# YuejiangDong/PPEA-Depth

Hardware: AMD Instinct MI355X
Metric: training img/s at 640x192 RepLKNet-31B (higher is better)
Workload: dtype bf16; 1 GPU; RepLKNet-31B Stage-1 640x192, 12 frame triplets/GPU, process_batch + backward + grad all-reduce + Adam; global_batch=12, per_gpu_batch=12, parallelism=dp1, use_checkpoint=BN-stat replay, no recompute (288 GB HBM), launch=whole step captured in one hipGraph

## Files before the change

### include/ppea_depth.h

```cpp
#ifndef PPEA_DEPTH_H
#define PPEA_DEPTH_H

#include <stdint.h>

#ifdef __cplusplus
extern "C" {
#endif

#define PPEA_ERR_UNSUPPORTED (-1)
#define PPEA_ERR_ARG (-2)

int ppea_abi_version(void);

int ppea_timestamp(void* slot, void* stream);

int ppea_dwconv_lk_fwd_f32(const float* x, const float* w_big, const float* w_small,
                           float* y_big, float* y_small,
                           int N, int C, int H, int W, int K, int KS, void* stream);
int ppea_dwconv_lk_fwd_bf16(const uint16_t* x, const float* w_big, const float* w_small,
                            uint16_t* y_big, uint16_t* y_small,
                            int N, int C, int H, int W, int K, int KS, void* stream);

int ppea_dwconv_lk_bwd_data_f32(const float* dy_big, const float* dy_small,
                                const float* w_big, const float* w_small, float* dx,
// ... 207 lines not shown
int ppea_ssim_l1_bwd_f32(const float* pred, const float* target, const float* d_out,
                         long dout_bstride, float* d_pred, int B, int C, int H, int W,
                         float alpha, void* stream);

int ppea_smooth_num_partials(void);
int ppea_smooth_fwd_f32(const float* disp, const float* img, float* partials,
                        int B, int C, int H, int W, void* stream);
int ppea_smooth_bwd_f32(const float* disp, const float* img, float gx, float gy, float* d_disp,
                        int B, int C, int H, int W, void* stream);

int ppea_loss_select_f32(const float* reproj, const float* identity, const float* warped_m1,
                         const float* warped_p1, const float* noise, float* sel,
                         uint8_t* src_idx, int64_t* frame_idx, int64_t* auto_idx,
                         int B, int C, int H, int W, int selec_reproj, void* stream);

int ppea_loss_tail_blocks(long total);
int ppea_loss_tail_fwd_f32(const float* sel, const int64_t* auto_idx, const float* cons, const float* aug, const float* multi,
                           const float* mono, float* mask, float* target, float* partial, float* out, int B, int H, int W,
                           int is_multi, void* stream);
int ppea_loss_tail_bwd_f32(const float* mask, const uint8_t* src, const float* out, const float* g_rl, const float* g_con,
                           const float* multi, const float* mono, float* d_reproj, float* d_multi, int B, int H, int W,
                           void* stream);

long ppea_conv_packed_bytes(int Cout, int Cin, int R, int S, int flip);
int ppea_conv_pack_weights(const void* w, int w_is_bf16, void* packed, int Cout, int Cin, int R, int S, int flip,
                           void* stream);
int ppea_conv_nhwc_bf16(const void* x, const void* w_packed, const void* bias, int bias_bf16, void* y,
                        int N, int H, int W, int Cin, int Cout, int R, int S, int stride, int pad, int reflect, int dil,
                        int Ho, int Wo, int act, int out_nchw, void* stream);
long ppea_conv_wgrad_workspace_bytes(int N, int Cin, int Cout, int R, int S, int stride, int Ho, int Wo);
int ppea_conv_wgrad_nhwc_bf16(const void* dz, const void* x, void* dw, int dw_bf16, void* workspace,
                              int N, int H, int W, int Cin, int Cout, int R, int S, int stride, int pad, int reflect,
                              int Ho, int Wo, void* stream);
int ppea_image_to_nhwc_bf16(const float* x, void* y, int N, int C, int H, int W, int Cp, float sub, float div,
                            void* stream);

int ppea_conv2d_f32_fwd(const float* x, const long* xs, const float* w, const float* bias, float* y, const long* ys, int N,
                        int Cin, int H, int W, int Cout, int R, int S, int stride, int pad, void* stream);
int ppea_conv2d_f32_dgrad(const float* dy, const long* dys, const float* w, float* dx, const long* dxs, int N, int Cin, int H,
                          int W, int Cout, int R, int S, int stride, int pad, int Ho, int Wo, void* stream);
long ppea_conv2d_f32_wgrad_workspace_bytes(int N, int Cin, int Cout, int R, int S, int Ho, int Wo);
int ppea_conv2d_f32_wgrad(const float* x, const long* xs, const float* dy, const long* dys, float* dw, float* workspace, int N,
                          int Cin, int H, int W, int Cout, int R, int S, int stride, int pad, int Ho, int Wo, void* stream);
int ppea_conv2d_bf16_fwd(const void* x, const long* xs, const void* w, const float* bias, void* y, const long* ys, int N,
                         int Cin, int H, int W, int Cout, int R, int S, int stride, int pad, void* stream);
int ppea_conv2d_bf16_dgrad(const void* dy, const long* dys, const void* w, void* dx, const long* dxs, int N, int Cin, int H,
                           int W, int Cout, int R, int S, int stride, int pad, int Ho, int Wo, void* stream);
int ppea_conv2d_bf16_wgrad(const void* x, const long* xs, const void* dy, const long* dys, float* dw, float* workspace, int N,
                           int Cin, int H, int W, int Cout, int R, int S, int stride, int pad, int Ho, int Wo, void* stream);

int ppea_nhwc_maxpool3x3s2_fwd_f32(const void* x, void* y, void* idx, int N, int H, int W, int C, void* stream);
int ppea_nhwc_maxpool3x3s2_fwd_bf16(const void* x, void* y, void* idx, int N, int H, int W, int C, void* stream);
int ppea_nhwc_maxpool3x3s2_bwd_f32(const void* dy, const void* idx, void* dx, int N, int H, int W, int C, void* stream);
int ppea_nhwc_maxpool3x3s2_bwd_bf16(const void* dy, const void* idx, void* dx, int N, int H, int W, int C, void* stream);

long ppea_conv_image_packed_bytes(int Cout, int K);
int ppea_conv_image_pack_weights(const void* w, int w_is_bf16, void* packed, int Cout, int Cin, int K, void* stream);
int ppea_conv_image_bf16(const void* x, const void* w_packed, void* y, int N, int H, int W, int Cout, int K, int stride,
                         int pad, int Ho, int Wo, int out_nchw, void* stream);
long ppea_conv_image_wgrad_workspace_bytes(int N, int Cout, int K, int Ho, int Wo);
int ppea_conv_image_wgrad_bf16(const void* dz, const void* x, void* dw, int dw_bf16, void* workspace, int N, int H, int W,
                               int Cin, int Cout, int K, int stride, int pad, int Ho, int Wo, void* stream);

int ppea_cost_volume_multi_fwd_f32(const float* cur, const float* lookup, const float* P, const float* inv_K,
                                   const float* bins, const int32_t* skip, float* cost, int B, int F, int C, int h, int w,
                                   int D, float eps, void* stream);
// ... 76 lines not shown
```

### ppea-depth_amd/csrc/common.h

```cpp
#pragma once
#include <hip/hip_runtime.h>
#include <stdint.h>

#define PPEA_ABI_VERSION 19
#define PPEA_ERR_UNSUPPORTED (-1)
#define PPEA_ERR_ARG (-2)
#define WAVE 64

__device__ __forceinline__ float bf16_to_f32(uint16_t v) {
    return __uint_as_float(((uint32_t)v) << 16);
}
__device__ __forceinline__ uint16_t f32_to_bf16(float f) {
    uint32_t u = __float_as_uint(f);
    if ((u & 0x7fffffffu) > 0x7f800000u) return (uint16_t)((u >> 16) | 0x40u);
    u += 0x7fffu + ((u >> 16) & 1u);
    return (uint16_t)(u >> 16);
}

template <typename T> __device__ __forceinline__ float ld_f32(const T* p);
template <> __device__ __forceinline__ float ld_f32<float>(const float* p) { return *p; }
template <> __device__ __forceinline__ float ld_f32<uint16_t>(const uint16_t* p) { return bf16_to_f32(*p); }
template <typename T> __device__ __forceinline__ void st_f32(T* p, float v);
template <> __device__ __forceinline__ void st_f32<float>(float* p, float v) { *p = v; }
template <> __device__ __forceinline__ void st_f32<uint16_t>(uint16_t* p, float v) { *p = f32_to_bf16(v); }

__device__ __forceinline__ float wave_sum(float v) {
#pragma unroll
    for (int o = 32; o > 0; o >>= 1) v += __shfl_xor(v, o, WAVE);
    return v;
}

static inline int launch_status() { return (int)hipGetLastError(); }
```

### ppea-depth_amd/csrc/conv_nhwc.hip

```cpp
#include "common.h"
#include <cstdlib>

namespace {

typedef __attribute__((ext_vector_type(8))) __bf16 bf16x8;
typedef __attribute__((ext_vector_type(4))) float f32x4;

constexpr int TILE_PX = 128;
constexpr int PITCH = 64;
__device__ __forceinline__ int swz_chunk(int row) { return ((row >> 2) & 1) << 1; }
constexpr int halo_cap(int stride, int ks) {
    return ks <= 3 ? (stride == 1 ? 4 * 66 : 9 * 65) : (stride == 1 ? 14 * 22 : 21 * 37);
}

__device__ __forceinline__ float bf2f(uint16_t v) { return __builtin_bit_cast(float, (uint32_t)v << 16); }
__device__ __forceinline__ uint16_t f2bf(float v) { return __builtin_bit_cast(uint16_t, (__bf16)v); }

struct ConvArgs {
    const uint16_t* x;
    const uint16_t* w;
    const void* bias;
    uint16_t* y;
    int N, H, W, Cin, CinP, Cout, stride, pad, reflect, dil, Ho, Wo, act, bias_bf16;
    int TR, TC, tiles_x, tiles_y;
};

enum { ACT_NONE = 0, ACT_RELU = 1, ACT_ELU = 2, ACT_SIGMOID = 3 };

template <int BN, int WM, int WN, int STRIDE, bool OUT_NCHW, int KS, int RPS = 1>
__global__ __launch_bounds__(256, 2) void conv_nhwc_kernel(const ConvArgs a) {
    static_assert(WM * WN == 4, "four waves");
    static_assert(RPS == 1 || RPS == KS, "one filter row or all of them per step");
    constexpr int MAX_A = (halo_cap(STRIDE, KS) * 4 + 255) / 256, MAX_B = (RPS * KS * BN * 4 + 255) / 256;
    constexpr int MT = 8 / WM;
    constexpr int NT = BN / 16 / WN;
    extern __shared__ __attribute__((aligned(16))) uint8_t lds[];

    const int TR = a.TR, TC = a.TC;
    const int HALO_H = (TR - 1) * STRIDE + KS, HALO_W = (TC - 1) * STRIDE + KS;
    const int halo_px = HALO_H * HALO_W;
    uint8_t* ldsA = lds;
    uint8_t* ldsB = lds + ((halo_px * PITCH + 127) / 128) * 128;

    const int tid = threadIdx.x, lane = tid & 63, wave = tid >> 6;
    const int wm = wave / WN, wn = wave % WN;
    const int g = lane >> 4, li = lane & 15;
    const int co0 = blockIdx.x * BN;
    int t = blockIdx.y;
    const int tx = t % a.tiles_x; t /= a.tiles_x;
    const int ty = t % a.tiles_y;
    const int n = t / a.tiles_y;
    const int oh0 = ty * TR, ow0 = tx * TC;
    const int ih0 = oh0 * STRIDE - a.pad, iw0 = ow0 * STRIDE - a.pad;
    const int Hl = (a.H - 1) * a.dil + 1, Wl = (a.W - 1) * a.dil + 1;
    const uint16_t* xn = a.x + (long)n * a.H * a.W * a.Cin;

    f32x4 acc[MT][NT];
#pragma unroll
    for (int i = 0; i < MT; ++i)
#pragma unroll
        for (int j = 0; j < NT; ++j) acc[i][j] = {0.f, 0.f, 0.f, 0.f};

    const int a_chunks = halo_px * 4;
    int a_src[MAX_A];
// ... 32 lines not shown
#pragma unroll
        for (int c = 0; c < MAX_A; ++c) {
            const int q = tid + c * 256;
            if (q < a_chunks) *reinterpret_cast<uint4*>(ldsA + (q >> 2) * PITCH + (((q & 3) ^ swz_chunk(q >> 2)) << 4)) = a_reg[c];
        }
    };
    auto load_b = [&](int c0, int r) {
#pragma unroll
        for (int c = 0; c < MAX_B; ++c) {
            const int q = tid + c * 256;
            if (q < b_chunks) {
                const int row = q >> 2;
                const int s = row / BN, co = co0 + row % BN;
                b_reg[c] = co < a.Cout ? *reinterpret_cast<const uint4*>(
                                             a.w + ((long)(r * KS + s) * a.Cout + co) * a.CinP + c0 + (q & 3) * 8)
                                       : make_uint4(0, 0, 0, 0);
            }
        }
    };
    auto store_b = [&]() {
#pragma unroll
        for (int c = 0; c < MAX_B; ++c) {
            const int q = tid + c * 256;
            if (q < b_chunks) *reinterpret_cast<uint4*>(ldsB + (q >> 2) * PITCH + (((q & 3) ^ swz_chunk(q >> 2)) << 4)) = b_reg[c];
        }
    };

    int a_px[MT];
#pragma unroll
    for (int i = 0; i < MT; ++i) {
        int m = (wm * MT + i) * 16 + li;
        if (m >= TR * TC) m = 0;
        a_px[i] = (m / TC) * STRIDE * HALO_W + (m % TC) * STRIDE;
    }
    const int b_off = (wn * NT * 16 + li) * PITCH + ((g ^ swz_chunk(li)) << 4);

    constexpr int SPS = KS / RPS;
    const int steps = (a.CinP / 32) * SPS;
    load_a(0);
    load_b(0, 0);
    for (int st = 0; st < steps; ++st) {
        const int r0 = (st % SPS) * RPS;
        __syncthreads();
        store_b();
        if (r0 == 0) store_a();
        __syncthreads();
        const int nxt = st + 1;
        if (nxt < steps) {
            load_b((nxt / SPS) * 32, (nxt % SPS) * RPS);
            if ((nxt % SPS) == 0) load_a((nxt / SPS) * 32);
        }
#pragma unroll
        for (int rr = 0; rr < RPS; ++rr) {
            const int r = r0 + rr;
#pragma unroll
            for (int s = 0; s < KS; ++s) {
                bf16x8 af[MT], bfr[NT];
#pragma unroll
                for (int i = 0; i < MT; ++i) {
                    const int px = a_px[i] + r * HALO_W + s;
                    af[i] = __builtin_bit_cast(bf16x8, *reinterpret_cast<const uint4*>(ldsA + px * PITCH + ((g ^ swz_chunk(px)) << 4)));
                }
#pragma unroll
                for (int j = 0; j < NT; ++j)
                    bfr[j] = __builtin_bit_cast(bf16x8, *reinterpret_cast<const uint4*>(ldsB + b_off + ((rr * KS + s) * BN + j * 16) * PITCH));
#pragma unroll
                for (int i = 0; i < MT; ++i)
#pragma unroll
                    for (int j = 0; j < NT; ++j) {
                        if constexpr (OUT_NCHW)
                            acc[i][j] = __builtin_amdgcn_mfma_f32_16x16x32_bf16(af[i], bfr[j], acc[i][j], 0, 0, 0);
                        else
                            acc[i][j] = __builtin_amdgcn_mfma_f32_16x16x32_bf16(bfr[j], af[i], acc[i][j], 0, 0, 0);
                    }
            }
        }
    }

    auto activate = [&](float v) -> float {
        switch (a.act) {
            case ACT_RELU: return v > 0.f ? v : 0.f;
            case ACT_ELU: return v > 0.f ? v : (__expf(v) - 1.f);
            case ACT_SIGMOID: return 1.f / (1.f + __expf(-v));
            default: return v;
        }
    };
    auto bias_at = [&](int co) -> float {
        if (a.bias == nullptr) return 0.f;
        return a.bias_bf16 ? bf2f(reinterpret_cast<const uint16_t*>(a.bias)[co]) : reinterpret_cast<const float*>(a.bias)[co];
    };
#pragma unroll
    for (int i = 0; i < MT; ++i) {
#pragma unroll
        for (int j = 0; j < NT; ++j) {
            const int cb = co0 + (wn * NT + j) * 16;
            if constexpr (OUT_NCHW) {
                const int m0 = (wm * MT + i) * 16 + 4 * g;
                const int oh = oh0 + m0 / TC, ow = ow0 + m0 % TC, co = cb + li;
                if (m0 >= TR * TC || oh >= a.Ho || co >= a.Cout || ow >= a.Wo) continue;
                const float bv = bias_at(co);
                uint16_t* dst = a.y + (((long)n * a.Cout + co) * a.Ho + oh) * a.Wo + ow;
                uint16_t v[4];
#pragma unroll
                for (int e = 0; e < 4; ++e) v[e] = f2bf(activate(acc[i][j][e] + bv));
                if (ow + 3 < a.Wo && (a.Wo & 3) == 0) {
                    *reinterpret_cast<uint2*>(dst) = make_uint2(v[0] | ((uint32_t)v[1] << 16), v[2] | ((uint32_t)v[3] << 16));
                } else {
// ... 8 lines not shown
                uint16_t* dst = a.y + (((long)n * a.Ho + oh) * a.Wo + ow) * a.Cout + co;
                uint16_t v[4];
#pragma unroll
                for (int e = 0; e < 4; ++e) v[e] = (co + e < a.Cout) ? f2bf(activate(acc[i][j][e] + bias_at(co + e))) : 0;
                if (co + 3 < a.Cout && (a.Cout & 3) == 0) {
                    *reinterpret_cast<uint2*>(dst) = make_uint2(v[0] | ((uint32_t)v[1] << 16), v[2] | ((uint32_t)v[3] << 16));
                } else {
#pragma unroll
                    for (int e = 0; e < 4; ++e)
                        if (co + e < a.Cout) dst[e] = v[e];
                }
            }
        }
    }
}

void pick_tile(ConvArgs& a, int stride, int ks, bool nchw) {
    int best_tr = 8, best_tc = 16;
    long best = (long)((a.Ho + 7) / 8) * ((a.Wo + 15) / 16);
    const int cand[4][2] = {{4, 32}, {2, 64}, {a.Wo <= 64 ? TILE_PX / a.Wo : 0, a.Wo}, {0, 0}};
    for (int c = 0; c < 3; ++c) {
        int tr = cand[c][0], tc = cand[c][1];
        if (tr <= 0 || tc <= 0) continue;
        if (tr > a.Ho) tr = a.Ho;
        if (nchw && (tc & 3)) continue;
        if (((tr - 1) * stride + ks) * ((tc - 1) * stride + ks) > halo_cap(stride, ks)) continue;
        const long tiles = (long)((a.Ho + tr - 1) / tr) * ((a.Wo + tc - 1) / tc);
        if (tiles < best) { best = tiles; best_tr = tr; best_tc = tc; }
    }
    a.TR = best_tr; a.TC = best_tc;
    a.tiles_x = (a.Wo + a.TC - 1) / a.TC; a.tiles_y = (a.Ho + a.TR - 1) / a.TR;
}

template <int BN, int WM, int WN, int STRIDE, bool NCHW, int KS, int RPS = 1>
int launch_conv(const ConvArgs& a, hipStream_t st) {
    const int halo_px = ((a.TR - 1) * STRIDE + KS) * ((a.TC - 1) * STRIDE + KS);
    if (halo_px > halo_cap(STRIDE, KS)) return PPEA_ERR_UNSUPPORTED;
    if constexpr (RPS == 1 && KS == 3 && BN <= 64) {
        static const bool one_row = getenv("PPEA_CONV_RPS") != nullptr && getenv("PPEA_CONV_RPS")[0] == '1';
        if (!one_row && a.CinP >= 256) return launch_conv<BN, WM, WN, STRIDE, NCHW, KS, KS>(a, st);
    }
    const size_t smem = (size_t)((halo_px * PITCH + 127) / 128) * 128 + (size_t)RPS * KS * BN * PITCH;
    if (smem > 160 * 1024) return PPEA_ERR_UNSUPPORTED;
    auto kern = conv_nhwc_kernel<BN, WM, WN, STRIDE, NCHW, KS, RPS>;
    if (smem > 64 * 1024) {
        hipError_t e = hipFuncSetAttribute(reinterpret_cast<const void*>(kern), hipFuncAttributeMaxDynamicSharedMemorySize, (int)smem);
        if (e != hipSuccess) return (int)e;
    }
    const dim3 grid((a.Cout + BN - 1) / BN, (unsigned)((long)a.tiles_x * a.tiles_y * a.N));
    hipLaunchKernelGGL(kern, grid, dim3(256), smem, st, a);
    return launch_status();
}

template <int STRIDE, bool NCHW, int KS>
int dispatch_bn(const ConvArgs& a, hipStream_t st) {
    const long tiles = (long)a.tiles_x * a.tiles_y * a.N;
    if constexpr (KS <= 3) {
        if (a.Cout > 64 && tiles * ((a.Cout + 127) / 128) >= 512 && !(KS == 3 && a.CinP >= 256))
            return launch_conv<128, 2, 2, STRIDE, NCHW, KS>(a, st);
    }
    static const bool no_narrow = getenv("PPEA_CONV_NO_NARROW") != nullptr;
    if (a.Cout > 32 && (no_narrow || tiles * ((a.Cout + 63) / 64) >= 256)) return launch_conv<64, 2, 2, STRIDE, NCHW, KS>(a, st);
    return launch_conv<32, 4, 1, STRIDE, NCHW, KS>(a, st);
}

template <int STRIDE, bool NCHW>
int dispatch_conv(ConvArgs& a, int ks, hipStream_t st) {
    pick_tile(a, STRIDE, ks, NCHW);
    switch (ks) {
        case 1: return dispatch_bn<STRIDE, NCHW, 1>(a, st);
        case 3: return dispatch_bn<STRIDE, NCHW, 3>(a, st);
        case 7: return dispatch_bn<STRIDE, NCHW, 7>(a, st);
    }
    return PPEA_ERR_UNSUPPORTED;
}

template <int NTC, int SL>
__global__ __launch_bounds__(256) void conv3x3_resident_kernel(const ConvArgs a) {
    constexpr int TR = 8, TC = 16, HALO_W = TC + 2, HALO_PX = (TR + 2) * HALO_W;
    constexpr int CO_ROWS = NTC * 16, MT = 2;
    constexpr int W_BYTES = SL * 9 * CO_ROWS * PITCH, H_BYTES = SL * HALO_PX * PITCH;
    constexpr int A_CHUNKS = SL * HALO_PX * 4, MAX_A = (A_CHUNKS + 255) / 256;
    extern __shared__ __attribute__((aligned(16))) uint8_t lds[];
    uint8_t* ldsW = lds;
    uint8_t* ldsH = lds + W_BYTES;

    const int tid = threadIdx.x, lane = tid & 63, wave = tid >> 6;
    const int g = lane >> 4, li = lane & 15;
    const int tiles = a.tiles_x * a.tiles_y * a.N;

    for (int q = tid; q < SL * 9 * CO_ROWS * 4; q += 256) {
        const int c = q & 3, row = q >> 2;
        const int co = row % CO_ROWS, st = row / CO_ROWS, tap = st % 9, sl = st / 9;
        uint4 v = make_uint4(0, 0, 0, 0);
        if (co < a.Cout) v = *reinterpret_cast<const uint4*>(a.w + ((long)tap * a.Cout + co) * a.CinP + sl * 32 + c * 8);
        *reinterpret_cast<uint4*>(ldsW + row * PITCH + ((c ^ swz_chunk(co)) << 4)) = v;
    }

    typedef __attribute__((ext_vector_type(4))) int i32x4;
    const unsigned long xb = (unsigned long)a.x;
    const unsigned nbytes = (unsigned)((long)a.N * a.H * a.W * a.Cin * 2);
    i32x4 rs;
    rs[0] = __builtin_amdgcn_readfirstlane((int)(unsigned)(xb & 0xffffffffu));
    rs[1] = __builtin_amdgcn_readfirstlane((int)(unsigned)(xb >> 32));
    rs[2] = __builtin_amdgcn_readfirstlane((int)nbytes);
    rs[3] = __builtin_amdgcn_readfirstlane(0x00020000);
    typedef __attribute__((ext_vector_type(4))) unsigned int u32x4;
    u32x4 a_reg[MAX_A];
    auto load_halo = [&](int t) {
        const int tx = t % a.tiles_x, ty = (t / a.tiles_x) % a.tiles_y, n = t / (a.tiles_x * a.tiles_y);
// ... 29 lines not shown
            if (q < A_CHUNKS) {
                const int c = q & 3, rest = q >> 2, px = rest % HALO_PX;
                *reinterpret_cast<u32x4*>(buf + rest * PITCH + ((c ^ swz_chunk(px)) << 4)) = a_reg[k];
            }
        }
    };

    int a_px[MT];
#pragma unroll
    for (int i = 0; i < MT; ++i) a_px[i] = (wave * MT + i) * HALO_W + li;
    const int b_off = li * PITCH + ((g ^ swz_chunk(li)) << 4);

    float bias_r[NTC][4];
#pragma unroll
    for (int j = 0; j < NTC; ++j)
#pragma unroll
        for (int e = 0; e < 4; ++e) {
            const int co = j * 16 + 4 * g + e;
            bias_r[j][e] = 0.f;
            if (a.bias != nullptr && co < a.Cout)
                bias_r[j][e] = a.bias_bf16 ? bf2f(reinterpret_cast<const uint16_t*>(a.bias)[co])
                                           : reinterpret_cast<const float*>(a.bias)[co];
        }

    int t = blockIdx.x;
    load_halo(t);
    halo_wait();
    store_halo(ldsH);
    __syncthreads();
    int cur = 0;
    for (; t < tiles; t += gridDim.x) {
        const int tn = t + gridDim.x;
        if (tn < tiles) load_halo(tn);
        const uint8_t* hb = ldsH + cur * H_BYTES;
        f32x4 acc[MT][NTC];
#pragma unroll
        for (int i = 0; i < MT; ++i)
#pragma unroll
            for (int j = 0; j < NTC; ++j) acc[i][j] = {0.f, 0.f, 0.f, 0.f};
#pragma unroll
        for (int sl = 0; sl < SL; ++sl)
#pragma unroll
            for (int r = 0; r < 3; ++r)
#pragma unroll
                for (int s3 = 0; s3 < 3; ++s3) {
                    bf16x8 af[MT], bfr[NTC];
#pragma unroll
                    for (int i = 0; i < MT; ++i) {
                        const int px = a_px[i] + r * HALO_W + s3;
                        af[i] = __builtin_bit_cast(bf16x8, *reinterpret_cast<const uint4*>(
                                                               hb + (sl * HALO_PX + px) * PITCH + ((g ^ swz_chunk(px)) << 4)));
                    }
#pragma unroll
                    for (int j = 0; j < NTC; ++j)
                        bfr[j] = __builtin_bit_cast(bf16x8, *reinterpret_cast<const uint4*>(
                                                                ldsW + b_off + (((sl * 9 + r * 3 + s3) * NTC + j) * 16) * PITCH));
#pragma unroll
                    for (int i = 0; i < MT; ++i)
#pragma unroll
                        for (int j = 0; j < NTC; ++j)
                            acc[i][j] = __builtin_amdgcn_mfma_f32_16x16x32_bf16(bfr[j], af[i], acc[i][j], 0, 0, 0);
                }
        const int tx = t % a.tiles_x, ty = (t / a.tiles_x) % a.tiles_y, n = t / (a.tiles_x * a.tiles_y);
#pragma unroll
        for (int i = 0; i < MT; ++i) {
            const int oh = ty * TR + wave * MT + i, ow = tx * TC + li;
            if (oh >= a.Ho || ow >= a.Wo) continue;
            uint16_t* row = a.y + (((long)n * a.Ho + oh) * a.Wo + ow) * a.Cout;
#pragma unroll
            for (int j = 0; j < NTC; ++j) {
                const int co = j * 16 + 4 * g;
                if (co >= a.Cout) continue;
                uint16_t v[4];
#pragma unroll
                for (int e = 0; e < 4; ++e) {
                    float f = acc[i][j][e];
                    if (co + e < a.Cout) {
                        f += bias_r[j][e];
                        switch (a.act) {
                            case ACT_RELU: f = f > 0.f ? f : 0.f; break;
                            case ACT_ELU: f = f > 0.f ? f : (__expf(f) - 1.f); break;
                            case ACT_SIGMOID: f = 1.f / (1.f + __expf(-f)); break;
                            default: break;
                        }
                    }
                    v[e] = f2bf(f);
                }
                if (co + 3 < a.Cout && (a.Cout & 3) == 0) {
                    *reinterpret_cast<uint2*>(row + co) = make_uint2(v[0] | ((uint32_t)v[1] << 16), v[2] | ((uint32_t)v[3] << 16));
                } else {
#pragma unroll
                    for (int e = 0; e < 4; ++e)
                        if (co + e < a.Cout) row[co + e] = v[e];
                }
            }
        }
        if (tn < tiles) {
            halo_wait();
            store_halo(ldsH + (cur ^ 1) * H_BYTES);
        }
        __syncthreads();
        cur ^= 1;
    }
}

template <int NTC, int SL>
int launch_resident(ConvArgs a, hipStream_t st) {
    a.TR = 8; a.TC = 16;
    a.tiles_x = (a.Wo + 15) / 16; a.tiles_y = (a.Ho + 7) / 8;
    constexpr size_t smem = (size_t)SL * 9 * NTC * 16 * PITCH + 2 * (size_t)SL * 180 * PITCH;
    auto kern = conv3x3_resident_kernel<NTC, SL>;
    if (smem > 64 * 1024) {
        hipError_t e = hipFuncSetAttribute(reinterpret_cast<const void*>(kern), hipFuncAttributeMaxDynamicSharedMemorySize, (int)smem);
        if (e != hipSuccess) return (int)e;
    }
    const long tiles = (long)a.tiles_x * a.tiles_y * a.N;
    int per_cu = (int)((160 * 1024) / smem);
    per_cu = per_cu > 3 ? 3 : (per_cu < 1 ? 1 : per_cu);
    const long grid = tiles < 256L * per_cu ? tiles : 256L * per_cu;
    hipLaunchKernelGGL(kern, dim3((unsigned)grid), dim3(256), smem, st, a);
    return launch_status();
}

bool resident_ok(const ConvArgs& a, int ks, int out_nchw) {
    const long tiles = (long)((a.Wo + 15) / 16) * ((a.Ho + 7) / 8) * a.N;
    return ks == 3 && a.stride == 1 && a.dil == 1 && !out_nchw && a.CinP == 32 && a.Cout <= 64 && a.pad <= 2 && tiles >= 2048 &&
           (long)a.N * a.H * a.W * a.Cin * 2 < (1L << 31);
}

int dispatch_resident(const ConvArgs& a, hipStream_t st) {
    switch ((a.Cout + 15) / 16) {
        case 1: return launch_resident<1, 1>(a, st);
        case 2: return launch_resident<2, 1>(a, st);
        case 3: case 4: return launch_resident<4, 1>(a, st);
    }
    return PPEA_ERR_UNSUPPORTED;
}

template <typename T>
__global__ void conv_pack_kernel(const T* __restrict__ w, uint16_t* __restrict__ out, int Cout, int Cin, int RS, int flip) {
    const int rows = flip ? Cin : Cout, cols = flip ? Cout : Cin;
    const int colsP = (cols + 31) / 32 * 32;
    const long total = (long)RS * rows * colsP;
    for (long i = (long)blockIdx.x * blockDim.x + threadIdx.x; i < total; i += (long)gridDim.x * blockDim.x) {
        const int c = (int)(i % colsP);
        const int rw = (int)((i / colsP) % rows);
        const int tap = (int)(i / ((long)colsP * rows));
        float v = 0.f;
        if (c < cols) {
            const int co = flip ? c : rw, ci = flip ? rw : c;
            const int tp = flip ? RS - 1 - tap : tap;
            v = ld_f32<T>(w + ((long)co * Cin + ci) * RS + tp);
        }
        out[i] = f2bf(v);
    }
}

__global__ void image_to_nhwc_kernel(const float* __restrict__ x, uint16_t* __restrict__ y, long NHW, int HW, int C, int Cp,
                                     float sub, float div) {
    for (long i = (long)blockIdx.x * blockDim.x + threadIdx.x; i < NHW; i += (long)gridDim.x * blockDim.x) {
        const long n = i / HW, p = i % HW;
        for (int c = 0; c < Cp; ++c)
            y[i * Cp + c] = c < C ? f2bf((x[(n * C + c) * HW + p] - sub) / div) : (uint16_t)0;
    }
}

}
// ... 12 lines not shown
    if (Cout <= 0 || Cin <= 0 || R <= 0 || S <= 0) return PPEA_ERR_ARG;
    const long total = packed_elems(Cout, Cin, R, S, flip);
    const int blocks = (int)((total + 255) / 256 > 4096 ? 4096 : (total + 255) / 256);
    if (w_is_bf16)
        hipLaunchKernelGGL(conv_pack_kernel<uint16_t>, dim3(blocks), dim3(256), 0, (hipStream_t)stream,
                           (const uint16_t*)w, (uint16_t*)packed, Cout, Cin, R * S, flip);
    else
        hipLaunchKernelGGL(conv_pack_kernel<float>, dim3(blocks), dim3(256), 0, (hipStream_t)stream, (const float*)w,
                           (uint16_t*)packed, Cout, Cin, R * S, flip);
    return launch_status();
}

int ppea_image_to_nhwc_bf16(const float* x, void* y, int N, int C, int H, int W, int Cp, float sub, float div, void* stream) {
    if (N <= 0 || C <= 0 || Cp < C || (Cp % 8) != 0) return PPEA_ERR_ARG;
    const long NHW = (long)N * H * W;
    const int blocks = (int)((NHW + 255) / 256 > 8192 ? 8192 : (NHW + 255) / 256);
    hipLaunchKernelGGL(image_to_nhwc_kernel, dim3(blocks), dim3(256), 0, (hipStream_t)stream, x, (uint16_t*)y, NHW, H * W, C, Cp,
                       sub, div);
    return launch_status();
}

int ppea_conv_nhwc_bf16(const void* x, const void* w_packed, const void* bias, int bias_bf16, void* y, int N, int H, int W,
                        int Cin, int Cout, int R, int S, int stride, int pad, int reflect, int dil, int Ho, int Wo, int act,
                        int out_nchw, void* stream) {
    if (N <= 0 || H <= 0 || W <= 0 || Cin <= 0 || Cout <= 0 || Ho <= 0 || Wo <= 0) return PPEA_ERR_ARG;
    if ((Cin % 8) != 0 || R != S || (R != 1 && R != 3 && R != 7) || (stride != 1 && stride != 2) || dil < 1 || pad < 0)
        return PPEA_ERR_UNSUPPORTED;
    if (reflect && (pad > 1 || dil != 1 || H < 2 || W < 2)) return PPEA_ERR_UNSUPPORTED;
    if ((long)H * W * Cin >= (1L << 31)) return PPEA_ERR_UNSUPPORTED;
    ConvArgs a;
    a.x = (const uint16_t*)x; a.w = (const uint16_t*)w_packed; a.bias = bias; a.y = (uint16_t*)y;
    a.N = N; a.H = H; a.W = W; a.Cin = Cin; a.CinP = (Cin + 31) / 32 * 32; a.Cout = Cout;
    a.stride = stride; a.pad = pad; a.reflect = reflect; a.dil = dil; a.Ho = Ho; a.Wo = Wo; a.act = act;
    a.bias_bf16 = bias_bf16;
    hipStream_t st = (hipStream_t)stream;
    static const bool no_resident = getenv("PPEA_CONV_NO_RESIDENT") != nullptr;
    if (!no_resident && resident_ok(a, R, out_nchw)) return dispatch_resident(a, st);
    if (stride == 1) return out_nchw ? dispatch_conv<1, true>(a, R, st) : dispatch_conv<1, false>(a, R, st);
    return out_nchw ? dispatch_conv<2, true>(a, R, st) : dispatch_conv<2, false>(a, R, st);
}

}
```

### ppea-depth_amd/ppeadepth/_abi.py

```python
import ctypes
import os

import torch

_HERE = os.path.dirname(os.path.abspath(__file__))
LIB_PATH = os.path.join(os.path.dirname(_HERE), "libppea_depth.so")

ABI_VERSION = 19

_vp, _i, _l, _f = ctypes.c_void_p, ctypes.c_int, ctypes.c_long, ctypes.c_float

SIGNATURES = {
    "ppea_abi_version": [],
    "ppea_timestamp": [_vp, _vp],
    "ppea_dwconv_lk_fwd_f32": [_vp] * 5 + [_i] * 6 + [_vp],
    "ppea_dwconv_lk_fwd_bf16": [_vp] * 5 + [_i] * 6 + [_vp],
    "ppea_dwconv_lk_bwd_data_f32": [_vp] * 5 + [_i] * 6 + [_vp],
    "ppea_dwconv_lk_bwd_data_bf16": [_vp] * 5 + [_i] * 6 + [_vp],
    "ppea_dwconv_lk_bwd_filter_f32": [_vp] * 3 + [_i] * 5 + [_vp],
    "ppea_dwconv3x3_fwd_f32": [_vp, _vp, _vp, _i, _i, _i, _i, _i, _vp],
    "ppea_dwconv3x3_fwd_bf16": [_vp, _vp, _vp, _i, _i, _i, _i, _i, _vp],
    "ppea_dwconv3x3_bwd_data_f32": [_vp, _vp, _vp, _i, _i, _i, _i, _i, _vp],
    "ppea_dwconv3x3_bwd_data_bf16": [_vp, _vp, _vp, _i, _i, _i, _i, _i, _vp],
    "ppea_dwconv_lk_packed_bytes": [_i, _i],
    "ppea_dwconv_lk_pack_bf16": [_vp, _vp, _i, _i, _i, _vp],
    "ppea_dwconv_lk_fwd_bf16p": [_vp] * 5 + [_i] * 6 + [_vp],
    "ppea_dwconv_lk_bwd_data_bf16p": [_vp] * 5 + [_i] * 6 + [_vp],
    "ppea_dwconv_lk_fwd_bn_bf16p": [_vp] * 6 + [_i, _l, _vp, _vp, _f, _f] + [_vp] * 4 + [_i] * 6 + [_vp],
    "ppea_pwconv_bf16": [_vp, _vp, _vp, _vp, _i, _i, _i, _i, _vp],
    "ppea_pwconv_ex_bf16": [_vp, _vp, _vp, _i, _i, _vp, _vp, _vp, _i, _i, _i, _i, _i, _vp],
    "ppea_dwconv_lk_fwd_bias_act_bf16p": [_vp, _vp, _vp, _i, _vp, _i, _i, _i, _i, _i, _vp],
    "ppea_dwconv_lk_fwd_bias_act_f32": [_vp, _vp, _vp, _i, _vp, _i, _i, _i, _i, _i, _vp],
    "ppea_dwconv_lk_fwd_bias_act_bf16": [_vp, _vp, _vp, _i, _vp, _i, _i, _i, _i, _i, _vp],
    "ppea_dwconv3x3_fwd_affine_f32": [_vp, _vp, _vp, _vp, _i, _vp, _i, _i, _i, _i, _i, _vp],
    "ppea_dwconv3x3_fwd_affine_bf16": [_vp, _vp, _vp, _vp, _i, _vp, _i, _i, _i, _i, _i, _vp],
    "ppea_pwconv_infer_bf16": [_vp, _vp, _vp, _vp, _i, _vp, _vp, _f, _vp, _vp, _vp, _vp, _i, _i, _i, _i, _vp],
    "ppea_pwgrad_workspace_bytes": [_i, _i, _i, _i],
    "ppea_pwgrad_bf16": [_vp, _vp, _vp, _vp, _i, _i, _i, _i, _i, _vp],
    "ppea_pwgrad_ex_bf16": [_vp, _vp, _vp, _i, _i, _i, _i, _vp, _i, _i, _vp, _i, _i, _i, _vp],
    "ppea_pwgrad_pair_workspace_bytes": [_i, _vp, _vp, _i],
    "ppea_pwgrad_ex_pair_bf16": [_vp, _vp, _vp, _i, _vp, _vp, _i, _vp, _vp, _vp, _vp, _vp, _vp, _vp, _vp],
# ... 74 lines not shown
    "ppea_ssim_l1_fwd_f32": [_vp, _vp, _vp, _l] + [_i] * 4 + [_f, _vp],
    "ppea_ssim_l1_bwd_f32": [_vp, _vp, _vp, _l, _vp] + [_i] * 4 + [_f, _vp],
    "ppea_smooth_num_partials": [],
    "ppea_smooth_fwd_f32": [_vp] * 3 + [_i] * 4 + [_vp],
    "ppea_smooth_bwd_f32": [_vp, _vp, _f, _f, _vp] + [_i] * 4 + [_vp],
    "ppea_loss_select_f32": [_vp] * 9 + [_i] * 5 + [_vp],
    "ppea_bn_fwd_channel_f32": [_vp, _vp, _vp, _vp, _f, _f, _vp, _vp, _vp, _f, _vp, _i, _i, _i, _i, _vp],
    "ppea_bn_fwd_channel_bf16": [_vp, _vp, _vp, _vp, _f, _f, _vp, _vp, _vp, _f, _vp, _i, _i, _i, _i, _vp],
    "ppea_bn_fwd_channel_sums_f32": [_vp, _vp, _i, _vp, _vp, _f, _f, _vp, _vp, _vp, _f, _vp, _i, _i, _i, _i, _vp],
    "ppea_bn_fwd_channel_sums_bf16": [_vp, _vp, _i, _vp, _vp, _f, _f, _vp, _vp, _vp, _f, _vp, _i, _i, _i, _i, _vp],
    "ppea_bn_bwd_channel_f32": [_vp, _vp, _vp, _vp, _vp, _f, _vp, _vp, _vp, _vp, _i, _i, _i, _i, _vp],
    "ppea_bn_bwd_channel_bf16": [_vp, _vp, _vp, _vp, _vp, _f, _vp, _vp, _vp, _vp, _i, _i, _i, _i, _vp],
    "ppea_bn_fwd_channel_next_f32": [_vp, _vp, _vp, _f, _f, _vp, _vp, _vp, _f, _vp, _vp, _i, _i, _i, _vp],
    "ppea_bn_fwd_channel_next_bf16": [_vp, _vp, _vp, _f, _f, _vp, _vp, _vp, _f, _vp, _vp, _i, _i, _i, _vp],
    "ppea_bn_bwd_channel_next_f32": [_vp, _vp, _vp, _vp, _vp, _vp, _f, _vp, _vp, _vp, _i, _i, _i, _vp],
    "ppea_bn_bwd_channel_next_bf16": [_vp, _vp, _vp, _vp, _vp, _vp, _f, _vp, _vp, _vp, _i, _i, _i, _vp],
    "ppea_bn_bwd_channel_dup_f32": [_vp, _vp, _vp, _vp, _vp, _vp, _f, _vp, _vp, _vp, _vp, _i, _i, _i, _i, _vp],
    "ppea_bn_bwd_channel_dup_bf16": [_vp, _vp, _vp, _vp, _vp, _vp, _f, _vp, _vp, _vp, _vp, _i, _i, _i, _i, _vp],
    "ppea_bn_bwd_channel_next_dup_f32": [_vp, _vp, _vp, _vp, _vp, _vp, _vp, _f, _vp, _vp, _vp, _i, _i, _i, _vp],
    "ppea_bn_bwd_channel_next_dup_bf16": [_vp, _vp, _vp, _vp, _vp, _vp, _vp, _f, _vp, _vp, _vp, _i, _i, _i, _vp],
    "ppea_bn_bwd_reduce_final_dup_f32": [_vp, _vp, _vp, _vp, _vp, _vp, _vp, _vp, _i, _i, _i, _i, _vp],
    "ppea_bn_bwd_reduce_final_dup_bf16": [_vp, _vp, _vp, _vp, _vp, _vp, _vp, _vp, _i, _i, _i, _i, _vp],
    "ppea_conv_image_packed_bytes": [_i, _i],
    "ppea_conv_image_pack_weights": [_vp, _i, _vp, _i, _i, _i, _vp],
    "ppea_conv_image_bf16": [_vp, _vp, _vp] + [_i] * 10 + [_vp],
    "ppea_conv_image_wgrad_workspace_bytes": [_i] * 5,
    "ppea_conv_image_wgrad_bf16": [_vp, _vp, _vp, _i, _vp] + [_i] * 10 + [_vp],
    "ppea_conv_packed_bytes": [_i] * 5,
    "ppea_conv_pack_weights": [_vp, _i, _vp, _i, _i, _i, _i, _i, _vp],
    "ppea_image_to_nhwc_bf16": [_vp, _vp, _i, _i, _i, _i, _i, _f, _f, _vp],
    "ppea_conv_nhwc_bf16": [_vp, _vp, _vp, _i, _vp] + [_i] * 15 + [_vp],
    "ppea_conv_wgrad_workspace_bytes": [_i] * 8,
    "ppea_conv_wgrad_nhwc_bf16": [_vp, _vp, _vp, _i, _vp] + [_i] * 12 + [_vp],
    "ppea_nhwc_up2cat_fwd_f32": [_vp, _vp, _vp, _i, _i, _i, _i, _i, _vp],
    "ppea_nhwc_up2cat_fwd_bf16": [_vp, _vp, _vp, _i, _i, _i, _i, _i, _vp],
    "ppea_nhwc_up2cat_bwd_f32": [_vp, _vp, _vp, _i, _i, _i, _i, _i, _vp],
    "ppea_nhwc_up2cat_bwd_bf16": [_vp, _vp, _vp, _i, _i, _i, _i, _i, _vp],
    "ppea_dwconv_lk_stats_partials": [_i] * 6,
    "ppea_dwconv_lk_fwd_stats_bf16p": [_vp] * 6 + [_i] * 6 + [_vp],
    "ppea_pwconv_stats_partials": [_i] * 4,
    "ppea_pwconv_stats_bf16": [_vp] * 5 + [_i] * 4 + [_vp],
    "ppea_bn_finalize_sums_f32": [_vp, _i, _i, ctypes.c_long, _f, _f, _vp, _vp, _vp, _vp, _vp, _vp],
    "ppea_conv2d_f32_fwd": [_vp] * 6 + [_i] * 9 + [_vp],
    "ppea_conv2d_f32_dgrad": [_vp] * 5 + [_i] * 11 + [_vp],
    "ppea_conv2d_f32_wgrad_workspace_bytes": [_i] * 7,
    "ppea_conv2d_f32_wgrad": [_vp] * 6 + [_i] * 11 + [_vp],
    "ppea_conv2d_bf16_fwd": [_vp] * 6 + [_i] * 9 + [_vp],
    "ppea_conv2d_bf16_dgrad": [_vp] * 5 + [_i] * 11 + [_vp],
    "ppea_conv2d_bf16_wgrad": [_vp] * 6 + [_i] * 11 + [_vp],
    "ppea_nhwc_maxpool3x3s2_fwd_f32": [_vp, _vp, _vp, _i, _i, _i, _i, _vp],
    "ppea_nhwc_maxpool3x3s2_fwd_bf16": [_vp, _vp, _vp, _i, _i, _i, _i, _vp],
    "ppea_nhwc_maxpool3x3s2_bwd_f32": [_vp, _vp, _vp, _i, _i, _i, _i, _vp],
    "ppea_nhwc_maxpool3x3s2_bwd_bf16": [_vp, _vp, _vp, _i, _i, _i, _i, _vp],
    "ppea_loss_tail_blocks": [_l],
    "ppea_loss_tail_fwd_f32": [_vp] * 10 + [_i] * 4 + [_vp],
    "ppea_loss_tail_bwd_f32": [_vp] * 9 + [_i] * 3 + [_vp],
    "ppea_cost_volume_reduce_f32": [_vp] * 6 + [_i] * 4 + [_vp],
    "ppea_cost_volume_multi_fwd_f32": [_vp] * 7 + [_i] * 6 + [_f, _vp],
    "ppea_cost_volume_multi_fwd_bf16": [_vp] * 8 + [_i] * 6 + [_f, _vp],
    "ppea_cost_volume_ring_fwd_f32": [_vp] * 8 + [_i] * 6 + [_f, _vp],
    "ppea_cost_volume_ring_fwd_bf16": [_vp] * 8 + [_i] * 6 + [_f, _vp],
    "ppea_cv_ring_store_f32": [_vp] * 3 + [_i] * 5 + [_vp],
    "ppea_cv_ring_store_bf16": [_vp] * 3 + [_i] * 5 + [_vp],
    "ppea_cv_ring_advance": [_vp, _i, _i, _vp],
    "ppea_depth_errors_workspace_bytes": [_i, _l],
    "ppea_depth_errors_f32": [_vp, _vp, _l, _vp, _vp, _vp, _vp, _vp, _i, _i, _i, _l, _i, _i, _f, _vp],
# ... 61 lines not shown
```

### ppea-depth_amd/ppeadepth/ops.py

```python
import weakref

import torch

from . import _abi
from ._abi import PpeaKernelError, call, ptr, stream_ptr, try_call

_F32 = torch.float32
_BF16 = torch.bfloat16

PROFILE_DWCONV = None


PROFILE_REPLAY = {}


def _timed(kind, K, fn):
    if PROFILE_DWCONV is None or K != 31:
        return fn()
    PROFILE_REPLAY.setdefault(kind, fn)
    s, e = torch.cuda.Event(enable_timing=True), torch.cuda.Event(enable_timing=True)
    s.record()
    r = fn()
    e.record()
    PROFILE_DWCONV.append((kind, s, e))
# ... 2010 lines not shown
        return y

    @staticmethod
    def backward(ctx, dy):
        x, w, y = ctx.saved_tensors
        stride, pad, reflect, act, out_nchw, has_bias, bdt = ctx.cfg
        N, Cin, H, W = x.shape
        Cout, _, R, S = w.shape
        Ho, Wo = dy.shape[2], dy.shape[3]
        db = None
        if act == 2 and not out_nchw and _nhwc_c_ok(Cout):
            dy = dy.contiguous(memory_format=torch.channels_last).to(_BF16)
            slabs = _abi.lib.ppea_nhwc_bias_elu_slabs(N * Ho * Wo, Cout)
            partial = torch.empty(slabs, Cout, device=dy.device, dtype=_F32)
            dz = torch.empty_like(dy)
            call("ppea_nhwc_bias_elu_bwd_bf16", _raw(dy), _raw(y), _raw(dz), ptr(partial), N * Ho * Wo, Cout, stream_ptr())
            if has_bias and ctx.needs_input_grad[2]:
                db = partial.sum(0).to(bdt)
        else:
            if act == 1:
                dz = dy * (y > 0)
            elif act == 2:
                dz = dy * torch.where(y > 0, torch.ones_like(y), y + 1)
            elif act == 3:
                dz = dy * (y * (1 - y))
            else:
                dz = dy
            if has_bias and ctx.needs_input_grad[2]:
                db = dz.float().sum((0, 2, 3)).to(bdt)
            dz = _as_nhwc(dz.to(_BF16))
        dx = dw = None
        if ctx.needs_input_grad[0]:
            wt = _conv_packed(w, True)
            if reflect:
                dpad = conv_nhwc_raw(dz, wt, None, Cin, R, S, 1, R - 1, False, stride, Ho + R - 1, Wo + S - 1, 0, False)
                dx = torch.empty(N, Cin, H, W, device=dz.device, dtype=_BF16, memory_format=torch.channels_last)
                call("ppea_nhwc_reflect_pad1_bwd_bf16", _raw(dpad), _raw(dx), N, H, W, Cin, stream_ptr())
            else:
                dx = conv_nhwc_raw(dz, wt, None, Cin, R, S, 1, R - 1 - pad, False, stride, H, W, 0, False)
        if ctx.needs_input_grad[1]:
            if Cout % 8 != 0:
                raise _abi.PpeaKernelError("conv weight gradient: output channels must be a multiple of 8 "
                                           "(pad the layer, see conv2d_nhwc)")
            ws = torch.empty(_abi.lib.ppea_conv_wgrad_workspace_bytes(N, Cin, Cout, R, S, stride, Ho, Wo) // 4, device=dz.device,
                             dtype=_F32)
            gdt = w.dtype if w.dtype in (_BF16, _F32) else _F32
            dw = torch.empty(Cout, Cin, R, S, device=dz.device, dtype=gdt)
            call("ppea_conv_wgrad_nhwc_bf16", _raw(dz), _raw(x), ptr(dw), int(gdt == _BF16), ptr(ws), N, H, W, Cin, Cout, R, S,
                 stride, pad, int(reflect), Ho, Wo, stream_ptr())
        return dx, dw, db, None, None, None, None, None


def _image_packed(w):
    def build(w):
        Cout, Cin, K, _ = w.shape
        wd = _pack_source(w)
        buf = torch.empty(_abi.lib.ppea_conv_image_packed_bytes(Cout, K) // 2, dtype=_BF16, device=w.device)
        call("ppea_conv_image_pack_weights", ptr(wd), int(wd.dtype == _BF16), ptr(buf), Cout, Cin, K, stream_ptr())
        return buf
    return _weight_image(w, "image", build)


class _ConvImage(torch.autograd.Function):

    @staticmethod
    def forward(ctx, x, w, pad, out_nchw):
        N, _, H, W = x.shape
# ... 134 lines not shown
```

Measured before the change: 370.0 img/s.

## Fold reflect-pad backward into 3x3 conv data-gradient kernel

Adds a backward-mode variant of the NHWC conv and resident 3x3 kernels. It folds the reflect-padding gradient directly into the accumulators by applying extra masked MFMA taps on border tiles. This removes the padded intermediate gradient tensor and the separate reflect-pad backward kernel for 3x3 stride-1 reflect convs in the decoder. The cost is extra per-tap work on edge tiles and a small reorder of LDS loads in the main loop.

```diff
diff --git a/include/ppea_depth.h b/include/ppea_depth.h
--- a/include/ppea_depth.h
+++ b/include/ppea_depth.h
@@ -263,6 +263,8 @@
 int ppea_conv_wgrad_nhwc_bf16(const void* dz, const void* x, void* dw, int dw_bf16, void* workspace,
                               int N, int H, int W, int Cin, int Cout, int R, int S, int stride, int pad, int reflect,
                               int Ho, int Wo, void* stream);
+int ppea_conv_dgrad_reflect_nhwc_bf16(const void* dz, const void* w_packed, void* dx, int N, int H, int W, int C, int Cx,
+                                      void* stream);
 int ppea_image_to_nhwc_bf16(const float* x, void* y, int N, int C, int H, int W, int Cp, float sub, float div,
                             void* stream);
 
diff --git a/ppea-depth_amd/csrc/common.h b/ppea-depth_amd/csrc/common.h
--- a/ppea-depth_amd/csrc/common.h
+++ b/ppea-depth_amd/csrc/common.h
@@ -2,7 +2,7 @@
 #include <hip/hip_runtime.h>
 #include <stdint.h>
 
-#define PPEA_ABI_VERSION 19
+#define PPEA_ABI_VERSION 20
 #define PPEA_ERR_UNSUPPORTED (-1)
 #define PPEA_ERR_ARG (-2)
 #define WAVE 64
diff --git a/ppea-depth_amd/csrc/conv_nhwc.hip b/ppea-depth_amd/csrc/conv_nhwc.hip
--- a/ppea-depth_amd/csrc/conv_nhwc.hip
+++ b/ppea-depth_amd/csrc/conv_nhwc.hip
@@ -23,13 +23,17 @@
     uint16_t* y;
     int N, H, W, Cin, CinP, Cout, stride, pad, reflect, dil, Ho, Wo, act, bias_bf16;
     int TR, TC, tiles_x, tiles_y;
+    int fold;
 };
 
+__device__ __forceinline__ int fold_target(int k, int n) { return k == 2 ? 1 : (k == 0 ? n - 2 : -1); }
+
 enum { ACT_NONE = 0, ACT_RELU = 1, ACT_ELU = 2, ACT_SIGMOID = 3 };
 
-template <int BN, int WM, int WN, int STRIDE, bool OUT_NCHW, int KS, int RPS = 1>
+template <int BN, int WM, int WN, int STRIDE, bool OUT_NCHW, int KS, int RPS = 1, bool BWD = false>
 __global__ __launch_bounds__(256, 2) void conv_nhwc_kernel(const ConvArgs a) {
     static_assert(WM * WN == 4, "four waves");
+    static_assert(!BWD || (KS == 3 && STRIDE == 1 && !OUT_NCHW), "folding data gradient: 3x3, stride 1, channels-last");
     static_assert(RPS == 1 || RPS == KS, "one filter row or all of them per step");
     constexpr int MAX_A = (halo_cap(STRIDE, KS) * 4 + 255) / 256, MAX_B = (RPS * KS * BN * 4 + 255) / 256;
     constexpr int MT = 8 / WM;
@@ -128,6 +132,17 @@
         int m = (wm * MT + i) * 16 + li;
         if (m >= TR * TC) m = 0;
         a_px[i] = (m / TC) * STRIDE * HALO_W + (m % TC) * STRIDE;
+    }
+    int a_hw[BWD ? MT : 1];
+    bool fold_tile = false;
+    if constexpr (BWD) {
+        fold_tile = a.fold && ((oh0 <= 1 && 1 < oh0 + TR) || (oh0 <= a.Ho - 2 && a.Ho - 2 < oh0 + TR) ||
+                               (ow0 <= 1 && 1 < ow0 + TC) || (ow0 <= a.Wo - 2 && a.Wo - 2 < ow0 + TC));
+#pragma unroll
+        for (int i = 0; i < MT; ++i) {
+            const int m = (wm * MT + i) * 16 + li;
+            a_hw[i] = ((oh0 + m / TC) << 16) | (ow0 + m % TC);
+        }
     }
     const int b_off = (wn * NT * 16 + li) * PITCH + ((g ^ swz_chunk(li)) << 4);
 
@@ -153,13 +168,13 @@
             for (int s = 0; s < KS; ++s) {
                 bf16x8 af[MT], bfr[NT];
 #pragma unroll
+                for (int j = 0; j < NT; ++j)
+                    bfr[j] = __builtin_bit_cast(bf16x8, *reinterpret_cast<const uint4*>(ldsB + b_off + ((rr * KS + s) * BN + j * 16) * PITCH));
+#pragma unroll
                 for (int i = 0; i < MT; ++i) {
                     const int px = a_px[i] + r * HALO_W + s;
                     af[i] = __builtin_bit_cast(bf16x8, *reinterpret_cast<const uint4*>(ldsA + px * PITCH + ((g ^ swz_chunk(px)) << 4)));
                 }
-#pragma unroll
-                for (int j = 0; j < NT; ++j)
-                    bfr[j] = __builtin_bit_cast(bf16x8, *reinterpret_cast<const uint4*>(ldsB + b_off + ((rr * KS + s) * BN + j * 16) * PITCH));
 #pragma unroll
                 for (int i = 0; i < MT; ++i)
 #pragma unroll
@@ -169,6 +184,34 @@
                         else
                             acc[i][j] = __builtin_amdgcn_mfma_f32_16x16x32_bf16(bfr[j], af[i], acc[i][j], 0, 0, 0);
                     }
+            }
+        }
+        if constexpr (BWD) {
+            if (fold_tile) {
+#pragma unroll 1
+                for (int e = 0; e < RPS * KS * 3; ++e) {
+                    const int rr = e / (KS * 3), s = (e / 3) % KS, v = e % 3 + 1, r = r0 + rr;
+                    const int t_oh = fold_target(r, a.Ho), t_ow = fold_target(s, a.Wo);
+                    if ((v & 1) && !(t_oh >= oh0 && t_oh < oh0 + TR)) continue;
+                    if ((v & 2) && !(t_ow >= ow0 && t_ow < ow0 + TC)) continue;
+                    const int rp = (v & 1) ? 2 - r : r, sp = (v & 2) ? 2 - s : s;
+                    bf16x8 af[MT], bfr[NT];
+#pragma unroll
+                    for (int j = 0; j < NT; ++j)
+                        bfr[j] = __builtin_bit_cast(bf16x8, *reinterpret_cast<const uint4*>(ldsB + b_off + ((rr * KS + s) * BN + j * 16) * PITCH));
+#pragma unroll
+                    for (int i = 0; i < MT; ++i) {
+                        const int px = a_px[i] + rp * HALO_W + sp;
+                        uint4 u = *reinterpret_cast<const uint4*>(ldsA + px * PITCH + ((g ^ swz_chunk(px)) << 4));
+                        const bool keep = (!(v & 1) || (a_hw[i] >> 16) == t_oh) && (!(v & 2) || (a_hw[i] & 0xffff) == t_ow);
+                        if (!keep) u = make_uint4(0, 0, 0, 0);
+                        af[i] = __builtin_bit_cast(bf16x8, u);
+                    }
+#pragma unroll
+                    for (int i = 0; i < MT; ++i)
+#pragma unroll
+                        for (int j = 0; j < NT; ++j) acc[i][j] = __builtin_amdgcn_mfma_f32_16x16x32_bf16(bfr[j], af[i], acc[i][j], 0, 0, 0);
+                }
             }
         }
     }
@@ -243,17 +286,17 @@
     a.tiles_x = (a.Wo + a.TC - 1) / a.TC; a.tiles_y = (a.Ho + a.TR - 1) / a.TR;
 }
 
-template <int BN, int WM, int WN, int STRIDE, bool NCHW, int KS, int RPS = 1>
+template <int BN, int WM, int WN, int STRIDE, bool NCHW, int KS, int RPS = 1, bool BWD = false>
 int launch_conv(const ConvArgs& a, hipStream_t st) {
     const int halo_px = ((a.TR - 1) * STRIDE + KS) * ((a.TC - 1) * STRIDE + KS);
     if (halo_px > halo_cap(STRIDE, KS)) return PPEA_ERR_UNSUPPORTED;
     if constexpr (RPS == 1 && KS == 3 && BN <= 64) {
         static const bool one_row = getenv("PPEA_CONV_RPS") != nullptr && getenv("PPEA_CONV_RPS")[0] == '1';
-        if (!one_row && a.CinP >= 256) return launch_conv<BN, WM, WN, STRIDE, NCHW, KS, KS>(a, st);
+        if (!one_row && a.CinP >= 256) return launch_conv<BN, WM, WN, STRIDE, NCHW, KS, KS, BWD>(a, st);
     }
     const size_t smem = (size_t)((halo_px * PITCH + 127) / 128) * 128 + (size_t)RPS * KS * BN * PITCH;
     if (smem > 160 * 1024) return PPEA_ERR_UNSUPPORTED;
-    auto kern = conv_nhwc_kernel<BN, WM, WN, STRIDE, NCHW, KS, RPS>;
+    auto kern = conv_nhwc_kernel<BN, WM, WN, STRIDE, NCHW, KS, RPS, BWD>;
     if (smem > 64 * 1024) {
         hipError_t e = hipFuncSetAttribute(reinterpret_cast<const void*>(kern), hipFuncAttributeMaxDynamicSharedMemorySize, (int)smem);
         if (e != hipSuccess) return (int)e;
@@ -263,16 +306,16 @@
     return launch_status();
 }
 
-template <int STRIDE, bool NCHW, int KS>
+template <int STRIDE, bool NCHW, int KS, bool BWD = false>
 int dispatch_bn(const ConvArgs& a, hipStream_t st) {
     const long tiles = (long)a.tiles_x * a.tiles_y * a.N;
     if constexpr (KS <= 3) {
         if (a.Cout > 64 && tiles * ((a.Cout + 127) / 128) >= 512 && !(KS == 3 && a.CinP >= 256))
-            return launch_conv<128, 2, 2, STRIDE, NCHW, KS>(a, st);
+            return launch_conv<128, 2, 2, STRIDE, NCHW, KS, 1, BWD>(a, st);
     }
     static const bool no_narrow = getenv("PPEA_CONV_NO_NARROW") != nullptr;
-    if (a.Cout > 32 && (no_narrow || tiles * ((a.Cout + 63) / 64) >= 256)) return launch_conv<64, 2, 2, STRIDE, NCHW, KS>(a, st);
-    return launch_conv<32, 4, 1, STRIDE, NCHW, KS>(a, st);
+    if (a.Cout > 32 && (no_narrow || tiles * ((a.Cout + 63) / 64) >= 256)) return launch_conv<64, 2, 2, STRIDE, NCHW, KS, 1, BWD>(a, st);
+    return launch_conv<32, 4, 1, STRIDE, NCHW, KS, 1, BWD>(a, st);
 }
 
 template <int STRIDE, bool NCHW>
@@ -286,7 +329,7 @@
     return PPEA_ERR_UNSUPPORTED;
 }
 
-template <int NTC, int SL>
+template <int NTC, int SL, bool BWD = false>
 __global__ __launch_bounds__(256) void conv3x3_resident_kernel(const ConvArgs a) {
     constexpr int TR = 8, TC = 16, HALO_W = TC + 2, HALO_PX = (TR + 2) * HALO_W;
     constexpr int CO_ROWS = NTC * 16, MT = 2;
@@ -382,6 +425,7 @@
     for (; t < tiles; t += gridDim.x) {
         const int tn = t + gridDim.x;
         if (tn < tiles) load_halo(tn);
+        const int tx = t % a.tiles_x, ty = (t / a.tiles_x) % a.tiles_y, n = t / (a.tiles_x * a.tiles_y);
         const uint8_t* hb = ldsH + cur * H_BYTES;
         f32x4 acc[MT][NTC];
 #pragma unroll
@@ -395,6 +439,10 @@
 #pragma unroll
                 for (int s3 = 0; s3 < 3; ++s3) {
                     bf16x8 af[MT], bfr[NTC];
+#pragma unroll
+                    for (int j = 0; j < NTC; ++j)
+                        bfr[j] = __builtin_bit_cast(bf16x8, *reinterpret_cast<const uint4*>(
+                                                                ldsW + b_off + (((sl * 9 + r * 3 + s3) * NTC + j) * 16) * PITCH));
 #pragma unroll
                     for (int i = 0; i < MT; ++i) {
                         const int px = a_px[i] + r * HALO_W + s3;
@@ -402,16 +450,43 @@
                                                                hb + (sl * HALO_PX + px) * PITCH + ((g ^ swz_chunk(px)) << 4)));
                     }
 #pragma unroll
+                    for (int i = 0; i < MT; ++i)
+#pragma unroll
+                        for (int j = 0; j < NTC; ++j)
+                            acc[i][j] = __builtin_amdgcn_mfma_f32_16x16x32_bf16(bfr[j], af[i], acc[i][j], 0, 0, 0);
+                }
+        if constexpr (BWD) {
+            const bool fold_tile = a.fold && (ty == 0 || (ty * TR <= a.Ho - 2 && a.Ho - 2 < ty * TR + TR) ||
+                                              tx == 0 || (tx * TC <= a.Wo - 2 && a.Wo - 2 < tx * TC + TC));
+            if (fold_tile) {
+#pragma unroll 1
+                for (int e = 0; e < SL * 27; ++e) {
+                    const int sl = e / 27, r = (e / 9) % 3, s3 = (e / 3) % 3, v = e % 3 + 1;
+                    const int t_oh = fold_target(r, a.Ho), t_ow = fold_target(s3, a.Wo);
+                    if ((v & 1) && !(t_oh >= ty * TR && t_oh < ty * TR + TR)) continue;
+                    if ((v & 2) && !(t_ow >= tx * TC && t_ow < tx * TC + TC)) continue;
+                    const int rp = (v & 1) ? 2 - r : r, sp = (v & 2) ? 2 - s3 : s3;
+                    bf16x8 af[MT], bfr[NTC];
+#pragma unroll
                     for (int j = 0; j < NTC; ++j)
                         bfr[j] = __builtin_bit_cast(bf16x8, *reinterpret_cast<const uint4*>(
                                                                 ldsW + b_off + (((sl * 9 + r * 3 + s3) * NTC + j) * 16) * PITCH));
 #pragma unroll
+                    for (int i = 0; i < MT; ++i) {
+                        const int px = a_px[i] + rp * HALO_W + sp;
+                        uint4 u = *reinterpret_cast<const uint4*>(hb + (sl * HALO_PX + px) * PITCH + ((g ^ swz_chunk(px)) << 4));
+                        const bool keep = (!(v & 1) || ty * TR + wave * MT + i == t_oh) && (!(v & 2) || tx * TC + li == t_ow);
+                        if (!keep) u = make_uint4(0, 0, 0, 0);
+                        af[i] = __builtin_bit_cast(bf16x8, u);
+                    }
+#pragma unroll
                     for (int i = 0; i < MT; ++i)
 #pragma unroll
                         for (int j = 0; j < NTC; ++j)
                             acc[i][j] = __builtin_amdgcn_mfma_f32_16x16x32_bf16(bfr[j], af[i], acc[i][j], 0, 0, 0);
                 }
-        const int tx = t % a.tiles_x, ty = (t / a.tiles_x) % a.tiles_y, n = t / (a.tiles_x * a.tiles_y);
+            }
+        }
 #pragma unroll
         for (int i = 0; i < MT; ++i) {
             const int oh = ty * TR + wave * MT + i, ow = tx * TC + li;
@@ -454,12 +529,12 @@
     }
 }
 
-template <int NTC, int SL>
+template <int NTC, int SL, bool BWD = false>
 int launch_resident(ConvArgs a, hipStream_t st) {
     a.TR = 8; a.TC = 16;
     a.tiles_x = (a.Wo + 15) / 16; a.tiles_y = (a.Ho + 7) / 8;
     constexpr size_t smem = (size_t)SL * 9 * NTC * 16 * PITCH + 2 * (size_t)SL * 180 * PITCH;
-    auto kern = conv3x3_resident_kernel<NTC, SL>;
+    auto kern = conv3x3_resident_kernel<NTC, SL, BWD>;
     if (smem > 64 * 1024) {
         hipError_t e = hipFuncSetAttribute(reinterpret_cast<const void*>(kern), hipFuncAttributeMaxDynamicSharedMemorySize, (int)smem);
         if (e != hipSuccess) return (int)e;
@@ -478,11 +553,12 @@
            (long)a.N * a.H * a.W * a.Cin * 2 < (1L << 31);
 }
 
+template <bool BWD = false>
 int dispatch_resident(const ConvArgs& a, hipStream_t st) {
     switch ((a.Cout + 15) / 16) {
-        case 1: return launch_resident<1, 1>(a, st);
-        case 2: return launch_resident<2, 1>(a, st);
-        case 3: case 4: return launch_resident<4, 1>(a, st);
+        case 1: return launch_resident<1, 1, BWD>(a, st);
+        case 2: return launch_resident<2, 1, BWD>(a, st);
+        case 3: case 4: return launch_resident<4, 1, BWD>(a, st);
     }
     return PPEA_ERR_UNSUPPORTED;
 }
@@ -561,7 +637,7 @@
     a.x = (const uint16_t*)x; a.w = (const uint16_t*)w_packed; a.bias = bias; a.y = (uint16_t*)y;
     a.N = N; a.H = H; a.W = W; a.Cin = Cin; a.CinP = (Cin + 31) / 32 * 32; a.Cout = Cout;
     a.stride = stride; a.pad = pad; a.reflect = reflect; a.dil = dil; a.Ho = Ho; a.Wo = Wo; a.act = act;
-    a.bias_bf16 = bias_bf16;
+    a.bias_bf16 = bias_bf16; a.fold = 0;
     hipStream_t st = (hipStream_t)stream;
     static const bool no_resident = getenv("PPEA_CONV_NO_RESIDENT") != nullptr;
     if (!no_resident && resident_ok(a, R, out_nchw)) return dispatch_resident(a, st);
@@ -569,4 +645,19 @@
     return out_nchw ? dispatch_conv<2, true>(a, R, st) : dispatch_conv<2, false>(a, R, st);
 }
 
-}
+int ppea_conv_dgrad_reflect_nhwc_bf16(const void* dz, const void* w_packed, void* dx, int N, int H, int W, int C, int Cx,
+                                      void* stream) {
+    if (N <= 0 || H <= 0 || W <= 0 || C <= 0 || Cx <= 0 || !dz || !dx || !w_packed) return PPEA_ERR_ARG;
+    if ((C % 8) != 0 || H < 3 || W < 3 || (long)H * W * C >= (1L << 31)) return PPEA_ERR_UNSUPPORTED;
+    ConvArgs a;
+    a.x = (const uint16_t*)dz; a.w = (const uint16_t*)w_packed; a.bias = nullptr; a.y = (uint16_t*)dx;
+    a.N = N; a.H = H; a.W = W; a.Cin = C; a.CinP = (C + 31) / 32 * 32; a.Cout = Cx;
+    a.stride = 1; a.pad = 1; a.reflect = 0; a.dil = 1; a.Ho = H; a.Wo = W; a.act = ACT_NONE; a.bias_bf16 = 0; a.fold = 1;
+    hipStream_t st = (hipStream_t)stream;
+    static const bool no_resident = getenv("PPEA_CONV_NO_RESIDENT") != nullptr;
+    if (!no_resident && resident_ok(a, 3, 0)) return dispatch_resident<true>(a, st);
+    pick_tile(a, 1, 3, false);
+    return dispatch_bn<1, false, 3, true>(a, st);
+}
+
+}
diff --git a/ppea-depth_amd/ppeadepth/_abi.py b/ppea-depth_amd/ppeadepth/_abi.py
--- a/ppea-depth_amd/ppeadepth/_abi.py
+++ b/ppea-depth_amd/ppeadepth/_abi.py
@@ -6,7 +6,7 @@
 _HERE = os.path.dirname(os.path.abspath(__file__))
 LIB_PATH = os.path.join(os.path.dirname(_HERE), "libppea_depth.so")
 
-ABI_VERSION = 19
+ABI_VERSION = 20
 
 _vp, _i, _l, _f = ctypes.c_void_p, ctypes.c_int, ctypes.c_long, ctypes.c_float
 
@@ -147,6 +147,7 @@
     "ppea_conv_nhwc_bf16": [_vp, _vp, _vp, _i, _vp] + [_i] * 15 + [_vp],
     "ppea_conv_wgrad_workspace_bytes": [_i] * 8,
     "ppea_conv_wgrad_nhwc_bf16": [_vp, _vp, _vp, _i, _vp] + [_i] * 12 + [_vp],
+    "ppea_conv_dgrad_reflect_nhwc_bf16": [_vp, _vp, _vp] + [_i] * 5 + [_vp],
     "ppea_nhwc_up2cat_fwd_f32": [_vp, _vp, _vp, _i, _i, _i, _i, _i, _vp],
     "ppea_nhwc_up2cat_fwd_bf16": [_vp, _vp, _vp, _i, _i, _i, _i, _i, _vp],
     "ppea_nhwc_up2cat_bwd_f32": [_vp, _vp, _vp, _i, _i, _i, _i, _i, _vp],
diff --git a/ppea-depth_amd/ppeadepth/ops.py b/ppea-depth_amd/ppeadepth/ops.py
--- a/ppea-depth_amd/ppeadepth/ops.py
+++ b/ppea-depth_amd/ppeadepth/ops.py
@@ -2066,7 +2066,10 @@
         dx = dw = None
         if ctx.needs_input_grad[0]:
             wt = _conv_packed(w, True)
-            if reflect:
+            if reflect and R == 3 and S == 3 and stride == 1 and pad == 1:
+                dx = torch.empty(N, Cin, H, W, device=dz.device, dtype=_BF16, memory_format=torch.channels_last)
+                call("ppea_conv_dgrad_reflect_nhwc_bf16", _raw(dz), ptr(wt), _raw(dx), N, H, W, Cout, Cin, stream_ptr())
+            elif reflect:
                 dpad = conv_nhwc_raw(dz, wt, None, Cin, R, S, 1, R - 1, False, stride, Ho + R - 1, Wo + S - 1, 0, False)
                 dx = torch.empty(N, Cin, H, W, device=dz.device, dtype=_BF16, memory_format=torch.channels_last)
                 call("ppea_nhwc_reflect_pad1_bwd_bf16", _raw(dpad), _raw(dx), N, H, W, Cin, stream_ptr())
```

New measurement: 364.1 img/s. 1.6% lower.
